# andrewmagis/snap-rnaseq

Measured on AMD Instinct MI355X. Metric: aligned reads/sec (100 bp SE, k=20 seed) at 1/2/4/8 GPUs + CPU baseline, higher is better.
Workload: dtype u8

## Files before the change

### snap-rnaseq_amd/csrc/aligner.hip

```cpp
#include <hip/hip_runtime.h>

#include <chrono>
#include <functional>
#include <cmath>
#include <cstring>
#include <algorithm>
#include <atomic>
#include <mutex>
#include <string>
#include <thread>
#include <type_traits>
#include <vector>

#include <fcntl.h>
#include <sys/stat.h>
#include <unistd.h>

#include "align_device.h"
#include "align_score.h"
#include "seed_lookup.h"
#include "simple_align.h"
#include "cigar.h"
#include "internal.h"
#include "large_copy.h"
// ... 973 lines not shown
uint32_t packedCode(char c) {
    return c == 'A' ? 0u : c == 'C' ? 1u : c == 'G' ? 2u : c == 'T' ? 3u : 4u;
}

int hostMapq(double pAll, double pBest, int score, int popular) {
    if (pAll < pBest) pAll = pBest;
    if (pAll == pBest && popular == 0 && score < 5) return 70;
    double c = pBest / pAll;
    int base;
    if (c >= 1) base = 69;
    else { base = (int)(-10 * log10(1 - c)); if (base > 69) base = 69; }
    int pen = popular - 10;
    if (pen < 0) pen = 0;
    base -= pen / 2;
    return base < 0 ? 0 : base;
}

}

struct ChunkSlot {
    char *dBases = nullptr, *dQuals = nullptr;
    uint64_t *dOffsets = nullptr;
    uint32_t *dLengths = nullptr;
    uint64_t *hOffsets = nullptr;
    uint32_t *hLengths = nullptr;
    snapgpu_result_t *hOut = nullptr;
    hipEvent_t h2d = nullptr;
    hipEvent_t done = nullptr;
    bool pending = false;
    uint64_t seq = 0, chunkBegin = 0, chunkN = 0, chunkEv = 0;
    snapgpu_result_t *chunkOut = nullptr;
};

struct ExecLane {
    hipStream_t stream = nullptr;
    void *arena = nullptr;
    void *bigArena = nullptr;
    uint32_t *counter = nullptr;
    unsigned long long *lookupStats = nullptr;
    hipEvent_t done = nullptr;
    uint64_t capReads = 0, capBytes = 0;
    uint32_t *dDefer = nullptr;
    snapgpu_result_t *dOut = nullptr;
    SeedRec *dSeeds = nullptr;
    ChunkSlot slot[2];
    uint32_t nextSlot = 0;
    unsigned long long *hLookupStats = nullptr;
};

struct EvSet {
    hipEvent_t e[4] = {};
    uint32_t *hCounter = nullptr;
};

struct SamState {
    struct Buf { void *p = nullptr; uint64_t cap = 0; };
    Buf aux;
    Buf len, scans, start, sums, text, bad;
    Buf bases, quals;
    Buf res, ed, nOps, ops;
    Buf key, keySorted, iota, order, slotLen, sortTemp;
    bool sorted = false;
    samline::SortArgs sortArgs{};
    std::vector<char> hAux;
    uint64_t fullBytes = 0;
    bool idsCached = false;
    std::string cachedRg;
    bool cachedHasRg = false;
    uint64_t n = 0, textBound = 0;
    bool ran = false;
    hipEvent_t ev[5] = {};
    double downloadMs = 0;
};

// ... 32 lines not shown

struct snapgpu_aligner {
    int device = 0;
    const snapgpu_index_t *idx = nullptr;
    snapgpu_aligner_params_t p{};
    uint32_t *dOverflow = nullptr, *dPieces = nullptr;
    uint4 *dBuckets = nullptr;
    uint64_t *dBucketBase = nullptr;
    uint32_t *dBucketCount = nullptr;
    snapgpu_bucket_info_t bucketInfo{};
    char *dGenomeAlloc = nullptr;
    GPlane *dGPlanes = nullptr;
    const char *dGenome = nullptr;
    DevTables *dTab = nullptr;
    ExecLane lane[2];
    std::vector<EvSet> evs;
    uint64_t nEvUsed = 0;
    bool overlapKernels = true;
    bool streamOpen = false;
    uint64_t nextLane = 0;
    uint64_t chunkSeq = 0;
    hipStream_t copyStream = nullptr;
    hipStream_t sideStream = nullptr;
    std::chrono::steady_clock::time_point streamStart;
    uint64_t arenaElems = 0;
    uint64_t arenaCap = 0;
    int grid = 0, grid256 = 0, grid512 = 0, gridBig = 0;
    uint64_t chunkReads = 1u << 20;
    uint64_t residentChunk = 1u << 18;
    uint32_t radixMin = SKCAP + 1;
    bool simplePass = true;
    int gridSimple = 0;
    bool orderLong = true;
    uint32_t tripRead = 0xffffffffu;
    snapgpu_timing_t timing{};
    snapgpu_aligner_stats_t stats{};
    snapgpu_device_reads_t *lastReads = nullptr;
    bool pendingTiming = false;
    uint32_t *dDiag = nullptr;
    unsigned long long *dPhase = nullptr;
    double timeoutSec = 0;
    bool failed = false;
    hipError_t (*eventQuery)(hipEvent_t) = hipEventQuery;
    hipEvent_t cev[2] = {};
    hipEvent_t residentSideDone = nullptr;
    bool residentSidePending = false;
// ... 325 lines not shown
        for (;;) {
            const hipError_t q = a->eventQuery(ev);
            if (q == hipSuccess) break;
            if (q != hipErrorNotReady) HIPCHK(q);
            if (std::chrono::duration<double>(std::chrono::steady_clock::now() - t0).count() > a->timeoutSec) {
                a->failed = true;
                snapgpu::setError("align kernel did not finish within SNAPGPU_TIMEOUT_S; the aligner is unusable "
                                  "and its device buffers are not released (exit the process)");
                return SNAPGPU_EDEVICE;
            }
            std::this_thread::sleep_for(std::chrono::microseconds(200));
        }
    }
    HIPCHK(hipEventSynchronize(ev));
    return SNAPGPU_OK;
}

int waitLane(snapgpu_aligner_t *a, ExecLane &L) {
    if (a->failed) return waitEvent(a, nullptr);
    HIPCHK(hipEventRecord(L.done, L.stream));
    return waitEvent(a, L.done);
}

}

namespace snapgpu {
void *hostAlloc(size_t bytes, bool *pinned, bool zero) {
    *pinned = false;
    int nd = g_hostDevices.load();
    if (nd == -2) {
        if (hipGetDeviceCount(&nd) != hipSuccess) nd = 0;
        g_hostDevices = nd;
    }
    if (nd > 0 && bytes >= (1u << 20)) {
        void *p = nullptr;
        size_t cap = bytes;
        {
            std::lock_guard<std::mutex> lk(g_pinMu);
            int best = -1;
            for (size_t i = 0; i < g_pinParked.size(); i++)
                if (g_pinParked[i].second >= bytes && g_pinParked[i].second <= 2 * bytes &&
                    (best < 0 || g_pinParked[i].second < g_pinParked[(size_t)best].second))
                    best = (int)i;
            if (best >= 0) {
                p = g_pinParked[(size_t)best].first;
                cap = g_pinParked[(size_t)best].second;
// ... 114 lines not shown
                                   idx->genome->nBases, a->dBuckets, a->dBucketBase, 4 * total);
                unsigned long long info[4] = {0, 0, 0, 0};
                if (chk(hipGetLastError(), "bucket_place_kernel / bucket_fill_kernel") &&
                    chk(hipMemcpyAsync(info, dCnt, sizeof(info), hipMemcpyDeviceToHost, s0), "counts") &&
                    chk(hipStreamSynchronize(s0), "bucket image build")) {
                    if (info[2] || info[0] != keys) {
                        snapgpu::setError("bucket image: " + std::to_string(info[2]) + " keys found no bucket, " +
                                          std::to_string(info[0]) + " of " + std::to_string(keys) + " inserted");
                        rc = SNAPGPU_EDEVICE;
                    }
                    snapgpu_bucket_info_t &bi = a->bucketInfo;
                    bi.nBuckets = total; bi.nKeys = info[0]; bi.nSlots = nSlots;
                    bi.nOverflowBuckets = info[1]; bi.maxDisplacement = info[3]; bi.bytes = total * 64;
                }
            }
        }
    }
    devFree(a, dSlots); devFree(a, dTB); devFree(a, dTS); devFree(a, dCnt);
    a->bucketInfo.buildMs = std::chrono::duration<double, std::milli>(std::chrono::steady_clock::now() - t0).count();
    return rc;
}

static void freeLaneChunkBuffers(snapgpu_aligner_t *a, ExecLane &L) {
    devFree(a, L.dDefer); devFree(a, L.dOut); devFree(a, L.dSeeds);
    L.dDefer = nullptr; L.dOut = nullptr; L.dSeeds = nullptr;
    for (ChunkSlot &S : L.slot) {
        devFree(a, S.dBases); devFree(a, S.dQuals); devFree(a, S.dOffsets); devFree(a, S.dLengths);
        S.dBases = S.dQuals = nullptr; S.dOffsets = nullptr; S.dLengths = nullptr;
        if (!a->failed) { hostPinnedFree(S.hOffsets); hostPinnedFree(S.hLengths); hostPinnedFree(S.hOut); }
        S.hOffsets = nullptr; S.hLengths = nullptr; S.hOut = nullptr;
    }
    L.capReads = L.capBytes = 0;
}

void snapgpu_aligner_free(snapgpu_aligner_t *a) {
    if (!a) return;
    if (a->failed) {
        delete a;
        return;
    }
    hipSetDevice(a->device);
    for (auto &L : a->lane) if (L.stream) hipStreamSynchronize(L.stream);
    devFree(a, a->dBuckets); devFree(a, a->dOverflow); devFree(a, a->dPieces);
    devFree(a, a->dBucketBase); devFree(a, a->dBucketCount); devFree(a, a->dGenomeAlloc); devFree(a, a->dTab);
    devFree(a, a->dGPlanes); devFree(a, a->dPhase); devFree(a, a->dDiag);
    for (auto &L : a->lane) {
        freeLaneChunkBuffers(a, L);
        devFree(a, L.arena); devFree(a, L.bigArena); devFree(a, L.counter); devFree(a, L.lookupStats);
        hostPinnedFree(L.hLookupStats);
        if (L.done) hipEventDestroy(L.done);
        for (ChunkSlot &S : L.slot) {
            if (S.h2d) hipEventDestroy(S.h2d);
            if (S.done) hipEventDestroy(S.done);
        }
        if (L.stream) hipStreamDestroy(L.stream);
    }
    if (a->copyStream) { hipStreamSynchronize(a->copyStream); hipStreamDestroy(a->copyStream); }
    if (a->sideStream) { hipStreamSynchronize(a->sideStream); hipStreamDestroy(a->sideStream); }
    for (auto &v : a->evs) {
        for (auto &e : v.e) if (e) hipEventDestroy(e);
        hostPinnedFree(v.hCounter);
    }
    for (auto &e : a->cev) if (e) hipEventDestroy(e);
    if (a->residentSideDone) hipEventDestroy(a->residentSideDone);
    for (auto *b : {&a->cgIn, &a->cgOut}) devFree(a, b->p);
    for (auto &b : a->aux) devFree(a, b.p);
    hostPinnedFree(a->cgPin);
    hostPinnedFree(a->cgPinOut);
    samStateFree(a, a->samBatch);
    bamStateFree(a, a->bamBatch);
    bgzfStateFree(a, a->bgzfBatch);
    for (int k = 0; k < 2; k++) {
        if (!a->failed) hostPinnedFree(a->samPin[k]);
        if (a->samPinDone[k]) hipEventDestroy(a->samPinDone[k]);
    }
    for (auto *b : {&a->fq.text, &a->fq.counts, &a->fq.tileStart, &a->fq.sums, &a->fq.nl, &a->fq.rec, &a->fq.baseStart,
                    &a->fq.idStart, &a->fq.sums2, &a->fq.tot, &a->fq.ids})
        devFree(a, b->p);
    for (int k = 0; k < 2; k++) {
        if (!a->failed) hostPinnedFree(a->fq.pin[k]);
        if (a->fq.pinDone[k]) hipEventDestroy(a->fq.pinDone[k]);
    }
    for (auto &e : a->fq.ev) if (e) hipEventDestroy(e);
// ... 16 lines not shown
    a->device = device;
    a->idx = idx;
    a->p = *params;
    if (const char *t = getenv("SNAPGPU_TIMEOUT_S")) a->timeoutSec = atof(t);
    if (const char *t = getenv("SNAPGPU_CHUNK_READS"); t && atoll(t) > 0) a->chunkReads = (uint64_t)atoll(t);
    if (const char *t = getenv("SNAPGPU_RADIX_MIN"); t && atoll(t) > 0) a->radixMin = (uint32_t)atoll(t);
    if (const char *t = getenv("SNAPGPU_OVERLAP")) a->overlapKernels = atoi(t) != 0;
    if (const char *t = getenv("SNAPGPU_ORDER_LONG")) a->orderLong = atoi(t) != 0;
    if (const char *t = getenv("SNAPGPU_SIMPLE_PASS")) a->simplePass = atoi(t) != 0;
    auto fail = [&](const char *what, hipError_t e) {
        snapgpu::setError(std::string(what) + ": " + hipGetErrorString(e));
        snapgpu_aligner_free(a);
        return (snapgpu_aligner_t *)nullptr;
    };
    hipError_t e;
    if ((e = hipSetDevice(device)) != hipSuccess) return fail("hipSetDevice", e);
    for (auto &L : a->lane) {
        if ((e = hipStreamCreateWithFlags(&L.stream, hipStreamNonBlocking)) != hipSuccess) return fail("stream", e);
        if ((e = hipEventCreateWithFlags(&L.done, hipEventDisableTiming)) != hipSuccess) return fail("event", e);
        for (ChunkSlot &S : L.slot)
            if ((e = hipEventCreateWithFlags(&S.h2d, hipEventDisableTiming)) != hipSuccess ||
                (e = hipEventCreateWithFlags(&S.done, hipEventDisableTiming)) != hipSuccess)
                return fail("event", e);
        if ((e = hipMalloc(&L.counter, 64)) != hipSuccess) return fail("counter", e);
        if ((e = hipMalloc(&L.lookupStats, 1024 * sizeof(unsigned long long))) != hipSuccess) return fail("lookup stats", e);
        if ((e = hipHostMalloc(&L.hLookupStats, 1024 * sizeof(unsigned long long), hipHostMallocDefault)) != hipSuccess)
            return fail("pinned lookup stats", e);
    }
    if ((e = hipStreamCreateWithFlags(&a->copyStream, hipStreamNonBlocking)) != hipSuccess) return fail("stream", e);
    {
        int least = 0, greatest = 0;
        const char *t = getenv("SNAPGPU_SIDE_PRIORITY");
        const bool high = !(t && atoi(t) == 0) && hipDeviceGetStreamPriorityRange(&least, &greatest) == hipSuccess;
        if ((e = high ? hipStreamCreateWithPriority(&a->sideStream, hipStreamNonBlocking, greatest)
                      : hipStreamCreateWithFlags(&a->sideStream, hipStreamNonBlocking)) != hipSuccess) return fail("stream", e);
    }
    for (auto &ev : a->cev) if ((e = hipEventCreate(&ev)) != hipSuccess) return fail("event", e);
    if ((e = hipEventCreateWithFlags(&a->residentSideDone, hipEventDisableTiming)) != hipSuccess) return fail("event", e);
    hipStream_t s0 = a->stream();
    if ((e = hipMalloc(&a->dDiag, 4 * sizeof(uint32_t))) != hipSuccess) return fail("watchdog record", e);
    if ((e = hipMemsetAsync(a->dDiag, 0, 4 * sizeof(uint32_t), s0)) != hipSuccess) return fail("watchdog record", e);
    if ((e = ensureDeviceTables(device)) != hipSuccess) return fail("device tables", e);
    const uint32_t nBases = idx->genome->nBases;
    const size_t gbytes = kDevGuard + nBases + kDevGuard;
    if ((e = hipMalloc(&a->dGenomeAlloc, gbytes)) != hipSuccess) return fail("hipMalloc genome", e);
    if ((e = hipMemsetAsync(a->dGenomeAlloc, 'n', gbytes, s0)) != hipSuccess) return fail("genome guard", e);
    if (uploadLarge(s0, a->dGenomeAlloc + kDevGuard, idx->genome->bases(), nBases)) { snapgpu_aligner_free(a); return nullptr; }
    a->dGenome = a->dGenomeAlloc + kDevGuard;
    {
        const uint64_t span = (uint64_t)nBases + 2 * kDevGuard;
        const uint64_t nw = (span + 31) / 32 + 8;
        if ((e = hipMalloc(&a->dGPlanes, nw * sizeof(GPlane))) != hipSuccess) return fail("hipMalloc planes", e);
        hipLaunchKernelGGL(pack_planes_kernel, dim3((unsigned)((nw + 255) / 256)), dim3(256), 0, s0, a->dGenomeAlloc,
                           span, nw, a->dGPlanes);
        if ((e = hipGetLastError()) != hipSuccess) return fail("pack_planes_kernel", e);
    }
    if ((e = hipMalloc(&a->dOverflow, idx->overflow.size() * 4 + 16)) != hipSuccess) return fail("hipMalloc ovf", e);
    if (uploadLarge(s0, a->dOverflow, idx->overflow.data(), idx->overflow.size() * 4)) { snapgpu_aligner_free(a); return nullptr; }
// ... 133 lines not shown

struct AlignExt {
    const snapgpu_search_t *search = nullptr;
    uint32_t maxHitsToGet = 0;
    uint32_t *hitScratch = nullptr;
    int32_t *multiFound = nullptr;
    snapgpu_multi_hit_t *multiHits = nullptr;
};

struct PassIO {
    const char *bases, *quals;
    const uint64_t *offsets;
    const uint32_t *lengths;
    uint64_t n;
    snapgpu_result_t *out;
    uint32_t *defer;
    uint32_t *defer2;
    uint32_t *ovf;
    SeedRec *seeds;
    uint32_t maxLen;
};

static int launch_passes(snapgpu_aligner_t *a, int li, const PassIO &io, const AlignExt &x, EvSet &ev,
                         const EvSet *prev) {
    ExecLane &L = a->lane[li];
    if (io.n == 0) return SNAPGPU_OK;
    if (io.n > 0xffffffffull) { snapgpu::setError("batch too large"); return SNAPGPU_EINVAL; }
    KArgs A;
    memset(&A, 0, sizeof(A));
    const snapgpu_index_t *idx = a->idx;
    A.buckets = a->dBuckets; A.bucketBase = a->dBucketBase; A.bucketCount = a->dBucketCount; A.overflow = a->dOverflow;
    A.genome = a->dGenome; A.pieces = a->dPieces; A.nPieces = (int32_t)idx->genome->pieceOffsets.size();
    A.gpl = a->dGPlanes; A.hasIupac = idx->hasIupac ? 1u : 0u;
    A.phaseBuf = a->dPhase;
    A.diag = a->dDiag;
    A.nBases = idx->genome->nBases; A.seedLen = idx->seedLen; A.nTables = idx->nTables;
    A.padding = idx->genome->chromosomePadding;
    A.maxHits = a->p.maxHitsToConsider; A.maxK = a->p.maxK; A.maxReadSize = a->p.maxReadSize;
    A.maxSeedsCmd = a->p.maxSeedsToUse; A.seedCoverage = a->p.maxSeedCoverage; A.extra = a->p.extraSearchDepth;
    A.explore = a->p.explorePopularSeeds; A.stopOnFirst = a->p.stopOnFirstHit; A.kRows = 31;
    A.radixMin = a->radixMin;
    A.tripRead = a->tripRead;
    A.tab = a->dTab;
    A.bases = io.bases; A.quals = io.quals; A.offsets = io.offsets; A.lengths = io.lengths;
    A.nReads = (uint32_t)io.n; A.out = io.out;
    A.counter = L.counter; A.arena = L.arena; A.arenaElems = a->arenaCap;
    if (a->arenaCap < a->arenaElems) { A.ovfList = io.ovf; A.ovfCount = L.counter + 6; }
    A.deferList = io.defer; A.deferCount = L.counter + 2; A.readList = nullptr;
    A.forcedStats = L.counter + 10;
    A.search = x.search; A.maxHitsToGet = x.maxHitsToGet;
    A.hitSlot = x.maxHitsToGet < 512 ? x.maxHitsToGet : 512;
    A.hitStride = multiHitStride(x.maxHitsToGet);
    A.hitScratch = x.hitScratch; A.multiFound = x.multiFound; A.multiHits = x.multiHits;
    int grid = a->grid;
    if ((uint64_t)grid > io.n) grid = (int)io.n;
    (void)hipGetLastError();
    if (prev && !a->overlapKernels) HIPCHK(hipStreamWaitEvent(L.stream, prev->e[2], 0));
    HIPCHK(hipMemsetAsync(L.counter, 0, 64, L.stream));
    HIPCHK(hipMemsetAsync(io.out, 0xff, io.n * sizeof(snapgpu_result_t), L.stream));
    A.seedRecs = nullptr;
    A.longCount = L.counter + 5;
    A.orderTmp = a->orderLong && io.n < (1ull << 28) ? io.defer2 : nullptr;
    HIPCHK(hipEventRecord(ev.e[3], L.stream));
    hipLaunchKernelGGL(seed_lookup_kernel, dim3((unsigned)((io.n + 4 * LOOKUP_WAVES - 1) / (4 * LOOKUP_WAVES))),
                       dim3(64 * LOOKUP_WAVES), 0, L.stream, A, io.seeds,
                       L.lookupStats);
    HIPCHK(hipGetLastError());
    if (A.orderTmp && io.maxLen > 128) {
        hipLaunchKernelGGL(order_long_kernel, dim3(1), dim3(256), 0, L.stream, A.orderTmp, A.longCount, A.deferList);
        HIPCHK(hipGetLastError());
    }
    A.orderTmp = nullptr;
    A.seedRecs = reinterpret_cast<const uint4 *>(io.seeds);
    HIPCHK(hipEventRecord(ev.e[0], L.stream));
    const bool ext = x.search || x.maxHitsToGet;
    if (a->simplePass && !ext && !A.stopOnFirst && !A.explore && A.maxHits >= 1 && A.maxHits < 0xffffu && A.seedRecs &&
        !A.phaseBuf) {
        KArgs Q = A;
        Q.counter = L.counter + 8;
        int gridS = a->gridSimple;
        if ((uint64_t)gridS > io.n) gridS = (int)io.n;
        if ((uint64_t)gridS * SIMPLE_CHUNK > io.n) gridS = (int)((io.n + SIMPLE_CHUNK - 1) / SIMPLE_CHUNK);
        hipLaunchKernelGGL(simple_align_kernel, dim3(gridS), dim3(64), 0, L.stream, Q, io.defer2, L.counter + 9,
                           L.counter + 12, L.counter + 13);
        HIPCHK(hipGetLastError());
        A.readList = io.defer2; A.readCount = L.counter + 9;
    }
    if (ext) hipLaunchKernelGGL((align_kernel<128, true>), dim3(grid), dim3(64), 0, L.stream, A);
    else hipLaunchKernelGGL((align_kernel<128, false>), dim3(grid), dim3(64), 0, L.stream, A);
    HIPCHK(hipGetLastError());
    HIPCHK(hipEventRecord(ev.e[1], L.stream));
    A.readList = nullptr; A.readCount = nullptr;
    KArgs M = A;
    M.counter = L.counter + 3;
    M.readList = io.defer; M.readCount = L.counter + 2;
    M.deferList = io.defer2; M.deferCount = L.counter + 4;
    int grid256 = a->grid256;
    if ((uint64_t)grid256 > io.n) grid256 = (int)io.n;
    if (ext) hipLaunchKernelGGL((align_kernel<256, true>), dim3(grid256), dim3(64), 0, L.stream, M);
    else hipLaunchKernelGGL((align_kernel<256, false>), dim3(grid256), dim3(64), 0, L.stream, M);
    HIPCHK(hipGetLastError());
    KArgs B = A;
    B.counter = L.counter + 1;
    B.readList = io.defer2; B.readCount = L.counter + 4;
    B.deferList = nullptr; B.deferCount = nullptr;
    B.seedRecs = nullptr;
    int grid2 = a->grid512;
    if ((uint64_t)grid2 > io.n) grid2 = (int)io.n;
    if (ext) hipLaunchKernelGGL((align_kernel<512, true>), dim3(grid2), dim3(64), 0, L.stream, B);
    else hipLaunchKernelGGL((align_kernel<512, false>), dim3(grid2), dim3(64), 0, L.stream, B);
    HIPCHK(hipGetLastError());
    if (a->gridBig) {
        KArgs V = A;
        V.counter = L.counter + 7;
        V.readList = io.ovf; V.readCount = L.counter + 6;
        V.deferList = nullptr; V.deferCount = nullptr;
        V.ovfList = nullptr; V.ovfCount = nullptr;
        V.seedRecs = nullptr;
        V.arena = L.bigArena; V.arenaElems = a->arenaElems;
        int gridV = a->gridBig;
        if ((uint64_t)gridV > io.n) gridV = (int)io.n;
        if (ext) hipLaunchKernelGGL((align_kernel<512, true>), dim3(gridV), dim3(64), 0, L.stream, V);
        else hipLaunchKernelGGL((align_kernel<512, false>), dim3(gridV), dim3(64), 0, L.stream, V);
        HIPCHK(hipGetLastError());
    }
    HIPCHK(hipEventRecord(ev.e[2], L.stream));
    HIPCHK(hipMemcpyAsync(ev.hCounter, L.counter, 64, hipMemcpyDeviceToHost, L.stream));
    return SNAPGPU_OK;
}

static EvSet *nextEvSet(snapgpu_aligner_t *a) {
    if (a->nEvUsed == a->evs.size()) {
        EvSet v;
        for (auto &e : v.e)
            if (hipEventCreate(&e) != hipSuccess) { snapgpu::setError("hipEventCreate"); return nullptr; }
        if (hipHostMalloc(&v.hCounter, 64, hipHostMallocDefault) != hipSuccess) { snapgpu::setError("pinned counter"); return nullptr; }
        a->evs.push_back(v);
    }
    return &a->evs[a->nEvUsed++];
}

static int beginCall(snapgpu_aligner_t *a) {
    a->nEvUsed = 0;
    a->timing = snapgpu_timing_t{};
    for (auto &L : a->lane) HIPCHK(hipMemsetAsync(L.lookupStats, 0, 1024 * sizeof(unsigned long long), L.stream));
    HIPCHK(hipMemsetAsync(a->dDiag, 0, sizeof(uint32_t) * 4, a->lane[0].stream));
    HIPCHK(hipStreamSynchronize(a->lane[0].stream));
    return SNAPGPU_OK;
}

static double busyUnion(snapgpu_aligner_t *a, int from, int to) {
    std::vector<std::pair<float, float>> iv;
    const hipEvent_t ref = a->evs[0].e[3];
    for (uint64_t i = 0; i < a->nEvUsed; i++) {
        float b = 0, e = 0;
        if (hipEventElapsedTime(&b, ref, a->evs[i].e[from]) != hipSuccess ||
            hipEventElapsedTime(&e, ref, a->evs[i].e[to]) != hipSuccess) return -1;
        iv.emplace_back(b, e);
    }
    std::sort(iv.begin(), iv.end());
    double total = 0, cs = -1e30, ce = -1e30;
    for (auto &x : iv) {
        if (x.first > ce) { if (ce > cs) total += ce - cs; cs = x.first; ce = x.second; }
        else if (x.second > ce) ce = x.second;
    }
    if (ce > cs) total += ce - cs;
    return total;
}

static void accountBusy(snapgpu_aligner_t *a) {
    if (a->nEvUsed == 0) return;
    a->timing.mainKernelBusyMs = busyUnion(a, 0, 1);
    a->timing.lookupKernelBusyMs = busyUnion(a, 3, 0);
}

static int accountEvSet(snapgpu_aligner_t *a, const EvSet &v) {
    float ms = 0;
    HIPCHK(hipEventElapsedTime(&ms, v.e[0], v.e[1]));
    a->timing.mainKernelMs += ms;
    HIPCHK(hipEventElapsedTime(&ms, v.e[1], v.e[2]));
    a->timing.spillKernelMs += ms;
    HIPCHK(hipEventElapsedTime(&ms, v.e[3], v.e[0]));
    a->timing.lookupKernelMs += ms;
    a->timing.nLaunches++;
    a->timing.nSpilled += v.hCounter[2];
    a->timing.nByteReads += v.hCounter[4];
    a->timing.nArenaOverflow += v.hCounter[6];
    a->timing.nForcedSettled += v.hCounter[10];
    a->timing.nForcedLimitSpans += v.hCounter[11];
    a->timing.nSimpleBailed += v.hCounter[9];
    a->timing.nSimpleReads += v.hCounter[12];
    a->timing.nSimpleWide += v.hCounter[13];
    return SNAPGPU_OK;
}

int snapgpu_align_batch_wait(snapgpu_aligner_t *a);

static int launch_resident(snapgpu_aligner_t *a, snapgpu_device_reads_t *d, const AlignExt &x) {
    if (!a || !d) return SNAPGPU_EINVAL;
    if (a->failed) { snapgpu::setError("aligner failed earlier (device timeout)"); return SNAPGPU_EDEVICE; }
    HIPCHK(hipSetDevice(a->device));
    int rc = snapgpu_align_batch_wait(a);
    if (rc) return rc;
    rc = beginCall(a);
    if (rc) return rc;
    if (a->residentSidePending) {
        for (auto &L : a->lane) HIPCHK(hipStreamWaitEvent(L.stream, a->residentSideDone, 0));
        a->residentSidePending = false;
    }
    const bool ext = x.search || x.maxHitsToGet;
    const uint64_t n = d->n;
    const uint64_t nChunks = ext || n == 0 ? 1 : (n + a->residentChunk - 1) / a->residentChunk;
    const uint64_t per = (n + nChunks - 1) / nChunks;
    for (uint64_t c = 0; c < nChunks; c++) {
        const uint64_t b = c * per, m = std::min(n, b + per) - b;
        EvSet *ev = nextEvSet(a);
        if (!ev) return SNAPGPU_EDEVICE;
        PassIO io{d->dBases, d->dQuals, d->dOffsets + b, d->dLengths + b, m, d->dOut + b, d->dDefer + b,
                  d->dDefer + (n + 1) + b, d->dDefer + 2 * (n + 1) + b, d->dSeeds + b * SEEDS_PER_READ, d->maxLen};
        if ((rc = launch_passes(a, (int)(c & 1), io, x, *ev, c ? &a->evs[a->nEvUsed - 2] : nullptr))) return rc;
    }
    a->lastReads = d;
    a->pendingTiming = n > 0;
    return SNAPGPU_OK;
}

int snapgpu_align_resident(snapgpu_aligner_t *a, snapgpu_device_reads_t *d) { return launch_resident(a, d, AlignExt()); }

static void addLookupStats(snapgpu_timing_t &t, const unsigned long long *ls) {
    for (int i = 0; i < 256; i++) {
        t.lookupSeeds += ls[4 * i];
        t.lookupProbes += ls[4 * i + 1];
        t.lookupOverflowReads += ls[4 * i + 2];
    }
}

static int checkWatchdog(snapgpu_aligner_t *a) {
    uint32_t diag[4];
    HIPCHK(hipMemcpy(diag, a->dDiag, sizeof(diag), hipMemcpyDeviceToHost));
    if (diag[0]) {
        char msg[160];
        snprintf(msg, sizeof msg, "device watchdog tripped: code %u read %u detail %u", diag[0], diag[1], diag[2]);
        snapgpu::setError(msg);
        return SNAPGPU_EDEVICE;
    }
    return SNAPGPU_OK;
}

int snapgpu_synchronize(snapgpu_aligner_t *a) {
    if (!a) return SNAPGPU_EINVAL;
    if (a->failed) { snapgpu::setError("aligner failed earlier (device timeout)"); return SNAPGPU_EDEVICE; }
    HIPCHK(hipSetDevice(a->device));
    for (auto &L : a->lane) {
        const int rc = waitLane(a, L);
        if (rc) return rc;
    }
    if (a->pendingTiming) {
        a->timing = snapgpu_timing_t{};
        for (uint64_t i = 0; i < a->nEvUsed; i++) {
            const int rc = accountEvSet(a, a->evs[i]);
            if (rc) return rc;
        }
        accountBusy(a);
        std::vector<unsigned long long> ls(1024);
        for (auto &L : a->lane) {
            HIPCHK(hipMemcpy(ls.data(), L.lookupStats, 1024 * sizeof(unsigned long long), hipMemcpyDeviceToHost));
            addLookupStats(a->timing, ls.data());
        }
        a->pendingTiming = false;
        const int rc = checkWatchdog(a);
        if (rc) return rc;
    }
    return SNAPGPU_OK;
}

static int checkRecords(snapgpu_aligner_t *a, uint64_t unwritten, uint64_t firstUnwritten) {
    a->timing.nUnwritten += unwritten;
    if (!unwritten) return SNAPGPU_OK;
    if (int rc = checkWatchdog(a)) return rc;
// ... 24 lines not shown
    return checkRecords(a, unwritten, first);
}

int snapgpu_results_download(snapgpu_aligner_t *a, snapgpu_device_reads_t *d, snapgpu_result_t *out) {
    if (!a || !d || !out) return SNAPGPU_EINVAL;
    HIPCHK(hipSetDevice(a->device));
    int rc = snapgpu_synchronize(a);
    if (rc) return rc;
    HIPCHK(hipMemcpyAsync(out, d->dOut, d->n * sizeof(snapgpu_result_t), hipMemcpyDeviceToHost, a->stream()));
    HIPCHK(hipStreamSynchronize(a->stream()));
    auto t0 = std::chrono::steady_clock::now();
    a->timing.nMapqFixed = 0;
    a->timing.nNulReads = 0;
    a->timing.nUnwritten = 0;
    rc = finishRecords(a, out, d->n);
    a->timing.fixupMs = std::chrono::duration<double, std::milli>(std::chrono::steady_clock::now() - t0).count();
    return rc;
}

static int ensureLaneCapacity(snapgpu_aligner_t *a, ExecLane &L, uint64_t reads, uint64_t bytes) {
    if (reads <= L.capReads && bytes <= L.capBytes) return SNAPGPU_OK;
    int rc = waitLane(a, L);
    if (rc) return rc;
    freeLaneChunkBuffers(a, L);
    reads = std::max<uint64_t>(reads, 1024);
    const uint64_t cb = bytes + 512;
    for (ChunkSlot &S : L.slot) {
        HIPCHK(hipMalloc(&S.dBases, cb));
        HIPCHK(hipMalloc(&S.dQuals, cb));
        HIPCHK(hipMemsetAsync(S.dBases, 0, cb, a->copyStream));
        HIPCHK(hipMemsetAsync(S.dQuals, 0, cb, a->copyStream));
        HIPCHK(hipMalloc(&S.dOffsets, (reads + 1) * 8));
        HIPCHK(hipMalloc(&S.dLengths, (reads + 1) * 4));
        HIPCHK(hipHostMalloc(&S.hOffsets, (reads + 1) * 8, hipHostMallocDefault));
        HIPCHK(hipHostMalloc(&S.hLengths, (reads + 1) * 4, hipHostMallocDefault));
        HIPCHK(hipHostMalloc(&S.hOut, (reads + 1) * sizeof(snapgpu_result_t), hipHostMallocDefault));
    }
    HIPCHK(hipMalloc(&L.dDefer, 3 * (reads + 1) * 4));
    HIPCHK(hipMalloc(&L.dOut, (reads + 1) * sizeof(snapgpu_result_t)));
    HIPCHK(hipMalloc(&L.dSeeds, (reads + 8) * SEEDS_PER_READ * sizeof(SeedRec)));
    L.capReads = reads;
    L.capBytes = bytes;
    return SNAPGPU_OK;
}

static int finishChunk(snapgpu_aligner_t *a, ChunkSlot &L) {
    if (!L.pending) return SNAPGPU_OK;
    snapgpu_result_t *out = L.chunkOut;
    L.pending = false;
    int rc = waitEvent(a, L.done);
    if (rc) return rc;
    if ((rc = accountEvSet(a, a->evs[L.chunkEv]))) return rc;
    const auto t0 = std::chrono::steady_clock::now();
    const uint64_t n = L.chunkN;
    snapgpu_result_t *dst = out + L.chunkBegin;
    const unsigned nt = n >= 65536 ? snapgpu::hostThreads(4) : 1u;
    std::vector<snapgpu_aligner_stats_t> st(nt, snapgpu_aligner_stats_t{});
    std::vector<uint64_t> fixed(nt, 0), nul(nt, 0), unwritten(nt, 0), first(nt, 0);
    auto work = [&](unsigned t) {
        const uint64_t b = n * t / nt, e = n * (t + 1) / nt;
        memcpy(dst + b, L.hOut + b, (e - b) * sizeof(snapgpu_result_t));
        uint64_t lk = 0, sc = 0, ig = 0, tm = 0, fx = 0, nu = 0, uw = 0, f0 = 0;
        for (uint64_t i = b; i < e; i++) {
// ... 42 lines not shown

static int finishOldest(snapgpu_aligner_t *a, bool *any) {
    ChunkSlot *o = nullptr;
    for (auto &L : a->lane)
        for (ChunkSlot &S : L.slot)
            if (S.pending && (!o || S.seq < o->seq)) o = &S;
    *any = o != nullptr;
    return o ? finishChunk(a, *o) : SNAPGPU_OK;
}

static int finishAll(snapgpu_aligner_t *a) {
    for (bool any = true; any;) {
        const int rc = finishOldest(a, &any);
        if (rc) return rc;
    }
    return SNAPGPU_OK;
}

static void abandonChunks(snapgpu_aligner_t *a) {
    for (auto &L : a->lane) {
        for (ChunkSlot &S : L.slot) S.pending = false;
        if (!a->failed) waitLane(a, L);
    }
    if (!a->failed && a->copyStream) (void)hipStreamSynchronize(a->copyStream);
    a->streamOpen = false;
}

int snapgpu_align_batch_submit(snapgpu_aligner_t *a, const snapgpu_reads_t *reads, snapgpu_result_t *out) {
    if (!a || !reads || !out) return SNAPGPU_EINVAL;
    if (a->failed) { snapgpu::setError("aligner failed earlier (device timeout)"); return SNAPGPU_EDEVICE; }
    HIPCHK(hipSetDevice(a->device));
    int rc = SNAPGPU_OK;
    if (!a->streamOpen) {
        if (a->pendingTiming && (rc = snapgpu_synchronize(a))) return rc;
        if ((rc = beginCall(a))) return rc;
        a->streamOpen = true;
        a->streamStart = std::chrono::steady_clock::now();
    }
    const uint64_t n = reads->n;
    if (n == 0) return SNAPGPU_OK;
    const uint64_t nChunks = (n + a->chunkReads - 1) / a->chunkReads;
    const uint64_t per = (n + nChunks - 1) / nChunks;
    std::vector<uint64_t> lo(nChunks, ~0ull), hi(nChunks, 0);
    uint64_t maxSpan = 0;
    for (uint64_t c = 0; c < nChunks; c++) {
        for (uint64_t i = c * per; i < std::min(n, (c + 1) * per); i++) {
// ... 14 lines not shown
    for (uint64_t c = 0; c < nChunks && rc == SNAPGPU_OK; c++) {
        const int li = (int)(a->nextLane++ & 1);
        ExecLane &L = a->lane[li];
        ChunkSlot &S = L.slot[L.nextSlot];
        L.nextSlot ^= 1u;
        for (bool any = true; S.pending && any;)
            if ((rc = finishOldest(a, &any))) break;
        if (rc) break;
        const uint64_t b = c * per, m = std::min(n, b + per) - b;
        uint32_t maxLen = 0;
        for (uint64_t i = 0; i < m; i++) {
            S.hOffsets[i] = reads->offsets[b + i] - lo[c];
            const uint32_t ln = reads->lengths[b + i];
            S.hLengths[i] = ln;
            maxLen = std::max(maxLen, ln);
        }
        const uint64_t span = std::min(hi[c] + 64, std::max(hostEnd, hi[c])) - lo[c];
        hipStream_t cs = a->copyStream, s = L.stream;
        HIPBRK(hipMemcpyAsync(S.dBases, reads->bases + lo[c], span, hipMemcpyHostToDevice, cs));
        HIPBRK(hipMemcpyAsync(S.dQuals, reads->quals + lo[c], span, hipMemcpyHostToDevice, cs));
        HIPBRK(hipMemcpyAsync(S.dOffsets, S.hOffsets, m * 8, hipMemcpyHostToDevice, cs));
        HIPBRK(hipMemcpyAsync(S.dLengths, S.hLengths, m * 4, hipMemcpyHostToDevice, cs));
        HIPBRK(hipEventRecord(S.h2d, cs));
        HIPBRK(hipStreamWaitEvent(s, S.h2d, 0));
        PassIO io{S.dBases, S.dQuals, S.dOffsets, S.dLengths, m, L.dOut, L.dDefer, L.dDefer + (L.capReads + 1),
                  L.dDefer + 2 * (L.capReads + 1), L.dSeeds, maxLen};
        EvSet *ev = nextEvSet(a);
        if (!ev) { rc = SNAPGPU_EDEVICE; break; }
        if ((rc = launch_passes(a, li, io, AlignExt(), *ev, a->nEvUsed >= 2 ? &a->evs[a->nEvUsed - 2] : nullptr))) break;
        HIPBRK(hipMemcpyAsync(S.hOut, L.dOut, m * sizeof(snapgpu_result_t), hipMemcpyDeviceToHost, s));
        HIPBRK(hipEventRecord(S.done, s));
        S.pending = true;
        S.seq = a->chunkSeq++;
        S.chunkBegin = b;
        S.chunkN = m;
        S.chunkEv = a->nEvUsed - 1;
        S.chunkOut = out;
    }
    if (rc) abandonChunks(a);
    return rc;
}

int snapgpu_align_batch_wait(snapgpu_aligner_t *a) {
    if (!a) return SNAPGPU_EINVAL;
    if (!a->streamOpen) return a->failed ? SNAPGPU_EDEVICE : SNAPGPU_OK;
    HIPCHK(hipSetDevice(a->device));
    int rc = finishAll(a);
    a->streamOpen = false;
    if (rc) {
        abandonChunks(a);
        return rc;
    }
    accountBusy(a);
// ... 1733 lines not shown
            rc = SNAPGPU_EDEVICE;
        }
    }
    devFree(a, dS); devFree(a, dO); devFree(a, dL);
    return rc;
}

int snapgpu_aligner_bucket_info(const snapgpu_aligner_t *a, snapgpu_bucket_info_t *info) {
    if (!a || !info) return SNAPGPU_EINVAL;
    *info = a->bucketInfo;
    return SNAPGPU_OK;
}

int snapgpu_gather_peak(snapgpu_aligner_t *a, uint32_t nLoads, double *ms) {
    if (!a || !ms || nLoads == 0) return SNAPGPU_EINVAL;
    HIPCHK(hipSetDevice(a->device));
    const uint64_t nBk = a->bucketInfo.nBuckets;
    if (nBk == 0 || nBk >= (1ull << 32)) { snapgpu::setError("gather_peak: bucket count"); return SNAPGPU_EINVAL; }
    const unsigned grid = (nLoads + 1023) / 1024;
    float best = 0;
    for (int rep = 0; rep < 3; rep++) {
        HIPCHK(hipEventRecord(a->cev[0], a->stream()));
        hipLaunchKernelGGL(gather_peak_kernel, dim3(grid), dim3(256), 0, a->stream(), a->dBuckets, (uint32_t)nBk, nLoads,
                           0x5bd1e995u * (rep + 1), a->lane[0].counter + 8);
        HIPCHK(hipGetLastError());
        HIPCHK(hipEventRecord(a->cev[1], a->stream()));
        HIPCHK(hipEventSynchronize(a->cev[1]));
        float f = 0;
        HIPCHK(hipEventElapsedTime(&f, a->cev[0], a->cev[1]));
        if (rep == 0 || f < best) best = f;
    }
    *ms = best;
    return SNAPGPU_OK;
}

int snapgpu_copy_peak(snapgpu_aligner_t *a, uint64_t bytes, double *ms) {
    if (!a || !ms || bytes < 4096) return SNAPGPU_EINVAL;
    if (a->failed) return SNAPGPU_EDEVICE;
    HIPCHK(hipSetDevice(a->device));
    const uint64_t nw = bytes / 16 / 1024 * 1024;
    void *src = nullptr, *dst = nullptr;
    HIPCHK(hipMalloc(&src, nw * 16));
    if (hipMalloc(&dst, nw * 16) != hipSuccess) { devFree(a, src); snapgpu::setError("copy_peak: hipMalloc"); return SNAPGPU_ENOMEM; }
    hipDeviceProp_t prop;
    HIPCHK(hipGetDeviceProperties(&prop, a->device));
    const unsigned grid = (unsigned)prop.multiProcessorCount * 16;
    float best = 0;
// ... 54 lines not shown
```

Measured before the change: 62.57 million.

## Run seed lookup and simple pass on a shared front stream with per-slot buffers

Seed lookup, order_long and simple_align now run on a new shared front stream that waits on the chunk's H2D event. The main align passes stay on the lane streams and wait on the front stream through an event, so lookup for the next chunk can overlap alignment of the previous one. To make that safe, the output, defer and seed buffers move from each lane to each chunk slot, and the device counters move to each event set. Separately, the 256 and 512 align passes are skipped when the reads are at most 128 bp and the index has no IUPAC codes, removing two kernel launches for short reads. The cost is more device memory, extra event and stream synchronisation, and the front stream serialising lookup work across both lanes.

Result: faster. 65.06 million (median of 6 runs) (+4.0%).

```diff
diff --git a/snap-rnaseq_amd/csrc/aligner.hip b/snap-rnaseq_amd/csrc/aligner.hip
--- a/snap-rnaseq_amd/csrc/aligner.hip
+++ b/snap-rnaseq_amd/csrc/aligner.hip
@@ -1019,6 +1019,9 @@
     char *dBases = nullptr, *dQuals = nullptr;
     uint64_t *dOffsets = nullptr;
     uint32_t *dLengths = nullptr;
+    uint32_t *dDefer = nullptr;
+    snapgpu_result_t *dOut = nullptr;
+    SeedRec *dSeeds = nullptr;
     uint64_t *hOffsets = nullptr;
     uint32_t *hLengths = nullptr;
     snapgpu_result_t *hOut = nullptr;
@@ -1033,20 +1036,17 @@
     hipStream_t stream = nullptr;
     void *arena = nullptr;
     void *bigArena = nullptr;
-    uint32_t *counter = nullptr;
     unsigned long long *lookupStats = nullptr;
     hipEvent_t done = nullptr;
     uint64_t capReads = 0, capBytes = 0;
-    uint32_t *dDefer = nullptr;
-    snapgpu_result_t *dOut = nullptr;
-    SeedRec *dSeeds = nullptr;
     ChunkSlot slot[2];
     uint32_t nextSlot = 0;
     unsigned long long *hLookupStats = nullptr;
 };
 
 struct EvSet {
-    hipEvent_t e[4] = {};
+    hipEvent_t e[6] = {};
+    uint32_t *dCounter = nullptr;
     uint32_t *hCounter = nullptr;
 };
 
@@ -1125,6 +1125,9 @@
     uint64_t chunkSeq = 0;
     hipStream_t copyStream = nullptr;
     hipStream_t sideStream = nullptr;
+    hipStream_t frontStream = nullptr;
+    hipEvent_t frontDone = nullptr;
+    uint32_t *dSink = nullptr;
     std::chrono::steady_clock::time_point streamStart;
     uint64_t arenaElems = 0;
     uint64_t arenaCap = 0;
@@ -1496,6 +1499,12 @@
     return waitEvent(a, L.done);
 }
 
+int waitFront(snapgpu_aligner_t *a) {
+    if (a->failed) return waitEvent(a, nullptr);
+    HIPCHK(hipEventRecord(a->frontDone, a->frontStream));
+    return waitEvent(a, a->frontDone);
+}
+
 }
 
 namespace snapgpu {
@@ -1656,9 +1665,9 @@
 }
 
 static void freeLaneChunkBuffers(snapgpu_aligner_t *a, ExecLane &L) {
-    devFree(a, L.dDefer); devFree(a, L.dOut); devFree(a, L.dSeeds);
-    L.dDefer = nullptr; L.dOut = nullptr; L.dSeeds = nullptr;
     for (ChunkSlot &S : L.slot) {
+        devFree(a, S.dDefer); devFree(a, S.dOut); devFree(a, S.dSeeds);
+        S.dDefer = nullptr; S.dOut = nullptr; S.dSeeds = nullptr;
         devFree(a, S.dBases); devFree(a, S.dQuals); devFree(a, S.dOffsets); devFree(a, S.dLengths);
         S.dBases = S.dQuals = nullptr; S.dOffsets = nullptr; S.dLengths = nullptr;
         if (!a->failed) { hostPinnedFree(S.hOffsets); hostPinnedFree(S.hLengths); hostPinnedFree(S.hOut); }
@@ -1674,13 +1683,14 @@
         return;
     }
     hipSetDevice(a->device);
+    if (a->frontStream) hipStreamSynchronize(a->frontStream);
     for (auto &L : a->lane) if (L.stream) hipStreamSynchronize(L.stream);
     devFree(a, a->dBuckets); devFree(a, a->dOverflow); devFree(a, a->dPieces);
     devFree(a, a->dBucketBase); devFree(a, a->dBucketCount); devFree(a, a->dGenomeAlloc); devFree(a, a->dTab);
     devFree(a, a->dGPlanes); devFree(a, a->dPhase); devFree(a, a->dDiag);
     for (auto &L : a->lane) {
         freeLaneChunkBuffers(a, L);
-        devFree(a, L.arena); devFree(a, L.bigArena); devFree(a, L.counter); devFree(a, L.lookupStats);
+        devFree(a, L.arena); devFree(a, L.bigArena); devFree(a, L.lookupStats);
         hostPinnedFree(L.hLookupStats);
         if (L.done) hipEventDestroy(L.done);
         for (ChunkSlot &S : L.slot) {
@@ -1691,8 +1701,12 @@
     }
     if (a->copyStream) { hipStreamSynchronize(a->copyStream); hipStreamDestroy(a->copyStream); }
     if (a->sideStream) { hipStreamSynchronize(a->sideStream); hipStreamDestroy(a->sideStream); }
+    if (a->frontStream) hipStreamDestroy(a->frontStream);
+    if (a->frontDone) hipEventDestroy(a->frontDone);
+    devFree(a, a->dSink);
     for (auto &v : a->evs) {
         for (auto &e : v.e) if (e) hipEventDestroy(e);
+        devFree(a, v.dCounter);
         hostPinnedFree(v.hCounter);
     }
     for (auto &e : a->cev) if (e) hipEventDestroy(e);
@@ -1755,7 +1769,6 @@
             if ((e = hipEventCreateWithFlags(&S.h2d, hipEventDisableTiming)) != hipSuccess ||
                 (e = hipEventCreateWithFlags(&S.done, hipEventDisableTiming)) != hipSuccess)
                 return fail("event", e);
-        if ((e = hipMalloc(&L.counter, 64)) != hipSuccess) return fail("counter", e);
         if ((e = hipMalloc(&L.lookupStats, 1024 * sizeof(unsigned long long))) != hipSuccess) return fail("lookup stats", e);
         if ((e = hipHostMalloc(&L.hLookupStats, 1024 * sizeof(unsigned long long), hipHostMallocDefault)) != hipSuccess)
             return fail("pinned lookup stats", e);
@@ -1767,6 +1780,12 @@
         const bool high = !(t && atoi(t) == 0) && hipDeviceGetStreamPriorityRange(&least, &greatest) == hipSuccess;
         if ((e = high ? hipStreamCreateWithPriority(&a->sideStream, hipStreamNonBlocking, greatest)
                       : hipStreamCreateWithFlags(&a->sideStream, hipStreamNonBlocking)) != hipSuccess) return fail("stream", e);
+        const char *f = getenv("SNAPGPU_FRONT_PRIORITY");
+        const bool fhigh = f && atoi(f) != 0 && hipDeviceGetStreamPriorityRange(&least, &greatest) == hipSuccess;
+        if ((e = fhigh ? hipStreamCreateWithPriority(&a->frontStream, hipStreamNonBlocking, greatest)
+                       : hipStreamCreateWithFlags(&a->frontStream, hipStreamNonBlocking)) != hipSuccess) return fail("stream", e);
+        if ((e = hipEventCreateWithFlags(&a->frontDone, hipEventDisableTiming)) != hipSuccess) return fail("event", e);
+        if ((e = hipMalloc(&a->dSink, 64)) != hipSuccess) return fail("sink", e);
     }
     for (auto &ev : a->cev) if ((e = hipEventCreate(&ev)) != hipSuccess) return fail("event", e);
     if ((e = hipEventCreateWithFlags(&a->residentSideDone, hipEventDisableTiming)) != hipSuccess) return fail("event", e);
@@ -1946,8 +1965,10 @@
 };
 
 static int launch_passes(snapgpu_aligner_t *a, int li, const PassIO &io, const AlignExt &x, EvSet &ev,
-                         const EvSet *prev) {
+                         const EvSet *prev, hipEvent_t inputs = nullptr, bool front = true) {
     ExecLane &L = a->lane[li];
+    uint32_t *const cnt = ev.dCounter;
+    const hipStream_t fs = front ? a->frontStream : L.stream;
     if (io.n == 0) return SNAPGPU_OK;
     if (io.n > 0xffffffffull) { snapgpu::setError("batch too large"); return SNAPGPU_EINVAL; }
     KArgs A;
@@ -1968,10 +1989,10 @@
     A.tab = a->dTab;
     A.bases = io.bases; A.quals = io.quals; A.offsets = io.offsets; A.lengths = io.lengths;
     A.nReads = (uint32_t)io.n; A.out = io.out;
-    A.counter = L.counter; A.arena = L.arena; A.arenaElems = a->arenaCap;
-    if (a->arenaCap < a->arenaElems) { A.ovfList = io.ovf; A.ovfCount = L.counter + 6; }
-    A.deferList = io.defer; A.deferCount = L.counter + 2; A.readList = nullptr;
-    A.forcedStats = L.counter + 10;
+    A.counter = cnt; A.arena = L.arena; A.arenaElems = a->arenaCap;
+    if (a->arenaCap < a->arenaElems) { A.ovfList = io.ovf; A.ovfCount = cnt + 6; }
+    A.deferList = io.defer; A.deferCount = cnt + 2; A.readList = nullptr;
+    A.forcedStats = cnt + 10;
     A.search = x.search; A.maxHitsToGet = x.maxHitsToGet;
     A.hitSlot = x.maxHitsToGet < 512 ? x.maxHitsToGet : 512;
     A.hitStride = multiHitStride(x.maxHitsToGet);
@@ -1979,65 +2000,73 @@
     int grid = a->grid;
     if ((uint64_t)grid > io.n) grid = (int)io.n;
     (void)hipGetLastError();
-    if (prev && !a->overlapKernels) HIPCHK(hipStreamWaitEvent(L.stream, prev->e[2], 0));
-    HIPCHK(hipMemsetAsync(L.counter, 0, 64, L.stream));
-    HIPCHK(hipMemsetAsync(io.out, 0xff, io.n * sizeof(snapgpu_result_t), L.stream));
+    if (prev && !a->overlapKernels) HIPCHK(hipStreamWaitEvent(fs, prev->e[2], 0));
+    if (inputs) HIPCHK(hipStreamWaitEvent(fs, inputs, 0));
+    HIPCHK(hipMemsetAsync(cnt, 0, 64, fs));
+    HIPCHK(hipMemsetAsync(io.out, 0xff, io.n * sizeof(snapgpu_result_t), fs));
     A.seedRecs = nullptr;
-    A.longCount = L.counter + 5;
+    A.longCount = cnt + 5;
     A.orderTmp = a->orderLong && io.n < (1ull << 28) ? io.defer2 : nullptr;
-    HIPCHK(hipEventRecord(ev.e[3], L.stream));
+    HIPCHK(hipEventRecord(ev.e[3], fs));
     hipLaunchKernelGGL(seed_lookup_kernel, dim3((unsigned)((io.n + 4 * LOOKUP_WAVES - 1) / (4 * LOOKUP_WAVES))),
-                       dim3(64 * LOOKUP_WAVES), 0, L.stream, A, io.seeds,
+                       dim3(64 * LOOKUP_WAVES), 0, fs, A, io.seeds,
                        L.lookupStats);
     HIPCHK(hipGetLastError());
     if (A.orderTmp && io.maxLen > 128) {
-        hipLaunchKernelGGL(order_long_kernel, dim3(1), dim3(256), 0, L.stream, A.orderTmp, A.longCount, A.deferList);
+        hipLaunchKernelGGL(order_long_kernel, dim3(1), dim3(256), 0, fs, A.orderTmp, A.longCount, A.deferList);
         HIPCHK(hipGetLastError());
     }
     A.orderTmp = nullptr;
     A.seedRecs = reinterpret_cast<const uint4 *>(io.seeds);
-    HIPCHK(hipEventRecord(ev.e[0], L.stream));
+    HIPCHK(hipEventRecord(ev.e[0], fs));
     const bool ext = x.search || x.maxHitsToGet;
     if (a->simplePass && !ext && !A.stopOnFirst && !A.explore && A.maxHits >= 1 && A.maxHits < 0xffffu && A.seedRecs &&
         !A.phaseBuf) {
         KArgs Q = A;
-        Q.counter = L.counter + 8;
+        Q.counter = cnt + 8;
         int gridS = a->gridSimple;
         if ((uint64_t)gridS > io.n) gridS = (int)io.n;
         if ((uint64_t)gridS * SIMPLE_CHUNK > io.n) gridS = (int)((io.n + SIMPLE_CHUNK - 1) / SIMPLE_CHUNK);
-        hipLaunchKernelGGL(simple_align_kernel, dim3(gridS), dim3(64), 0, L.stream, Q, io.defer2, L.counter + 9,
-                           L.counter + 12, L.counter + 13);
+        hipLaunchKernelGGL(simple_align_kernel, dim3(gridS), dim3(64), 0, fs, Q, io.defer2, cnt + 9,
+                           cnt + 12, cnt + 13);
         HIPCHK(hipGetLastError());
-        A.readList = io.defer2; A.readCount = L.counter + 9;
-    }
+        A.readList = io.defer2; A.readCount = cnt + 9;
+    }
+    HIPCHK(hipEventRecord(ev.e[4], fs));
+    HIPCHK(hipStreamWaitEvent(L.stream, ev.e[4], 0));
+    HIPCHK(hipEventRecord(ev.e[5], L.stream));
     if (ext) hipLaunchKernelGGL((align_kernel<128, true>), dim3(grid), dim3(64), 0, L.stream, A);
     else hipLaunchKernelGGL((align_kernel<128, false>), dim3(grid), dim3(64), 0, L.stream, A);
     HIPCHK(hipGetLastError());
     HIPCHK(hipEventRecord(ev.e[1], L.stream));
     A.readList = nullptr; A.readCount = nullptr;
+    const bool pass2 = io.maxLen > 128 || idx->hasIupac;
+    const bool pass3 = pass2 && (io.maxLen > 256 || idx->hasIupac);
     KArgs M = A;
-    M.counter = L.counter + 3;
-    M.readList = io.defer; M.readCount = L.counter + 2;
-    M.deferList = io.defer2; M.deferCount = L.counter + 4;
+    M.counter = cnt + 3;
+    M.readList = io.defer; M.readCount = cnt + 2;
+    M.deferList = io.defer2; M.deferCount = cnt + 4;
     int grid256 = a->grid256;
     if ((uint64_t)grid256 > io.n) grid256 = (int)io.n;
-    if (ext) hipLaunchKernelGGL((align_kernel<256, true>), dim3(grid256), dim3(64), 0, L.stream, M);
+    if (!pass2) {}
+    else if (ext) hipLaunchKernelGGL((align_kernel<256, true>), dim3(grid256), dim3(64), 0, L.stream, M);
     else hipLaunchKernelGGL((align_kernel<256, false>), dim3(grid256), dim3(64), 0, L.stream, M);
     HIPCHK(hipGetLastError());
     KArgs B = A;
-    B.counter = L.counter + 1;
-    B.readList = io.defer2; B.readCount = L.counter + 4;
+    B.counter = cnt + 1;
+    B.readList = io.defer2; B.readCount = cnt + 4;
     B.deferList = nullptr; B.deferCount = nullptr;
     B.seedRecs = nullptr;
     int grid2 = a->grid512;
     if ((uint64_t)grid2 > io.n) grid2 = (int)io.n;
-    if (ext) hipLaunchKernelGGL((align_kernel<512, true>), dim3(grid2), dim3(64), 0, L.stream, B);
+    if (!pass3) {}
+    else if (ext) hipLaunchKernelGGL((align_kernel<512, true>), dim3(grid2), dim3(64), 0, L.stream, B);
     else hipLaunchKernelGGL((align_kernel<512, false>), dim3(grid2), dim3(64), 0, L.stream, B);
     HIPCHK(hipGetLastError());
     if (a->gridBig) {
         KArgs V = A;
-        V.counter = L.counter + 7;
-        V.readList = io.ovf; V.readCount = L.counter + 6;
+        V.counter = cnt + 7;
+        V.readList = io.ovf; V.readCount = cnt + 6;
         V.deferList = nullptr; V.deferCount = nullptr;
         V.ovfList = nullptr; V.ovfCount = nullptr;
         V.seedRecs = nullptr;
@@ -2049,7 +2078,7 @@
         HIPCHK(hipGetLastError());
     }
     HIPCHK(hipEventRecord(ev.e[2], L.stream));
-    HIPCHK(hipMemcpyAsync(ev.hCounter, L.counter, 64, hipMemcpyDeviceToHost, L.stream));
+    HIPCHK(hipMemcpyAsync(ev.hCounter, cnt, 64, hipMemcpyDeviceToHost, L.stream));
     return SNAPGPU_OK;
 }
 
@@ -2058,6 +2087,7 @@
         EvSet v;
         for (auto &e : v.e)
             if (hipEventCreate(&e) != hipSuccess) { snapgpu::setError("hipEventCreate"); return nullptr; }
+        if (hipMalloc(&v.dCounter, 64) != hipSuccess) { snapgpu::setError("device counter"); return nullptr; }
         if (hipHostMalloc(&v.hCounter, 64, hipHostMallocDefault) != hipSuccess) { snapgpu::setError("pinned counter"); return nullptr; }
         a->evs.push_back(v);
     }
@@ -2069,11 +2099,15 @@
     a->timing = snapgpu_timing_t{};
     for (auto &L : a->lane) HIPCHK(hipMemsetAsync(L.lookupStats, 0, 1024 * sizeof(unsigned long long), L.stream));
     HIPCHK(hipMemsetAsync(a->dDiag, 0, sizeof(uint32_t) * 4, a->lane[0].stream));
+    for (auto &L : a->lane) {
+        HIPCHK(hipEventRecord(L.done, L.stream));
+        HIPCHK(hipStreamWaitEvent(a->frontStream, L.done, 0));
+    }
     HIPCHK(hipStreamSynchronize(a->lane[0].stream));
     return SNAPGPU_OK;
 }
 
-static double busyUnion(snapgpu_aligner_t *a, int from, int to) {
+static double busyUnion(snapgpu_aligner_t *a, int from, int to, int from2 = -1, int to2 = -1) {
     std::vector<std::pair<float, float>> iv;
     const hipEvent_t ref = a->evs[0].e[3];
     for (uint64_t i = 0; i < a->nEvUsed; i++) {
@@ -2081,6 +2115,10 @@
         if (hipEventElapsedTime(&b, ref, a->evs[i].e[from]) != hipSuccess ||
             hipEventElapsedTime(&e, ref, a->evs[i].e[to]) != hipSuccess) return -1;
         iv.emplace_back(b, e);
+        if (from2 < 0) continue;
+        if (hipEventElapsedTime(&b, ref, a->evs[i].e[from2]) != hipSuccess ||
+            hipEventElapsedTime(&e, ref, a->evs[i].e[to2]) != hipSuccess) return -1;
+        iv.emplace_back(b, e);
     }
     std::sort(iv.begin(), iv.end());
     double total = 0, cs = -1e30, ce = -1e30;
@@ -2094,13 +2132,15 @@
 
 static void accountBusy(snapgpu_aligner_t *a) {
     if (a->nEvUsed == 0) return;
-    a->timing.mainKernelBusyMs = busyUnion(a, 0, 1);
+    a->timing.mainKernelBusyMs = busyUnion(a, 0, 4, 5, 1);
     a->timing.lookupKernelBusyMs = busyUnion(a, 3, 0);
 }
 
 static int accountEvSet(snapgpu_aligner_t *a, const EvSet &v) {
     float ms = 0;
-    HIPCHK(hipEventElapsedTime(&ms, v.e[0], v.e[1]));
+    HIPCHK(hipEventElapsedTime(&ms, v.e[0], v.e[4]));
+    a->timing.mainKernelMs += ms;
+    HIPCHK(hipEventElapsedTime(&ms, v.e[5], v.e[1]));
     a->timing.mainKernelMs += ms;
     HIPCHK(hipEventElapsedTime(&ms, v.e[1], v.e[2]));
     a->timing.spillKernelMs += ms;
@@ -2129,6 +2169,7 @@
     rc = beginCall(a);
     if (rc) return rc;
     if (a->residentSidePending) {
+        HIPCHK(hipStreamWaitEvent(a->frontStream, a->residentSideDone, 0));
         for (auto &L : a->lane) HIPCHK(hipStreamWaitEvent(L.stream, a->residentSideDone, 0));
         a->residentSidePending = false;
     }
@@ -2142,7 +2183,8 @@
         if (!ev) return SNAPGPU_EDEVICE;
         PassIO io{d->dBases, d->dQuals, d->dOffsets + b, d->dLengths + b, m, d->dOut + b, d->dDefer + b,
                   d->dDefer + (n + 1) + b, d->dDefer + 2 * (n + 1) + b, d->dSeeds + b * SEEDS_PER_READ, d->maxLen};
-        if ((rc = launch_passes(a, (int)(c & 1), io, x, *ev, c ? &a->evs[a->nEvUsed - 2] : nullptr))) return rc;
+        if ((rc = launch_passes(a, (int)(c & 1), io, x, *ev, c ? &a->evs[a->nEvUsed - 2] : nullptr, nullptr, false)))
+            return rc;
     }
     a->lastReads = d;
     a->pendingTiming = n > 0;
@@ -2179,6 +2221,7 @@
         const int rc = waitLane(a, L);
         if (rc) return rc;
     }
+    if (const int rc = waitFront(a)) return rc;
     if (a->pendingTiming) {
         a->timing = snapgpu_timing_t{};
         for (uint64_t i = 0; i < a->nEvUsed; i++) {
@@ -2249,6 +2292,7 @@
     if (reads <= L.capReads && bytes <= L.capBytes) return SNAPGPU_OK;
     int rc = waitLane(a, L);
     if (rc) return rc;
+    if ((rc = waitFront(a))) return rc;
     freeLaneChunkBuffers(a, L);
     reads = std::max<uint64_t>(reads, 1024);
     const uint64_t cb = bytes + 512;
@@ -2262,10 +2306,10 @@
         HIPCHK(hipHostMalloc(&S.hOffsets, (reads + 1) * 8, hipHostMallocDefault));
         HIPCHK(hipHostMalloc(&S.hLengths, (reads + 1) * 4, hipHostMallocDefault));
         HIPCHK(hipHostMalloc(&S.hOut, (reads + 1) * sizeof(snapgpu_result_t), hipHostMallocDefault));
-    }
-    HIPCHK(hipMalloc(&L.dDefer, 3 * (reads + 1) * 4));
-    HIPCHK(hipMalloc(&L.dOut, (reads + 1) * sizeof(snapgpu_result_t)));
-    HIPCHK(hipMalloc(&L.dSeeds, (reads + 8) * SEEDS_PER_READ * sizeof(SeedRec)));
+        HIPCHK(hipMalloc(&S.dDefer, 3 * (reads + 1) * 4));
+        HIPCHK(hipMalloc(&S.dOut, (reads + 1) * sizeof(snapgpu_result_t)));
+        HIPCHK(hipMalloc(&S.dSeeds, (reads + 8) * SEEDS_PER_READ * sizeof(SeedRec)));
+    }
     L.capReads = reads;
     L.capBytes = bytes;
     return SNAPGPU_OK;
@@ -2354,6 +2398,7 @@
         for (ChunkSlot &S : L.slot) S.pending = false;
         if (!a->failed) waitLane(a, L);
     }
+    if (!a->failed) waitFront(a);
     if (!a->failed && a->copyStream) (void)hipStreamSynchronize(a->copyStream);
     a->streamOpen = false;
 }
@@ -2414,13 +2459,12 @@
         HIPBRK(hipMemcpyAsync(S.dOffsets, S.hOffsets, m * 8, hipMemcpyHostToDevice, cs));
         HIPBRK(hipMemcpyAsync(S.dLengths, S.hLengths, m * 4, hipMemcpyHostToDevice, cs));
         HIPBRK(hipEventRecord(S.h2d, cs));
-        HIPBRK(hipStreamWaitEvent(s, S.h2d, 0));
-        PassIO io{S.dBases, S.dQuals, S.dOffsets, S.dLengths, m, L.dOut, L.dDefer, L.dDefer + (L.capReads + 1),
-                  L.dDefer + 2 * (L.capReads + 1), L.dSeeds, maxLen};
+        PassIO io{S.dBases, S.dQuals, S.dOffsets, S.dLengths, m, S.dOut, S.dDefer, S.dDefer + (L.capReads + 1),
+                  S.dDefer + 2 * (L.capReads + 1), S.dSeeds, maxLen};
         EvSet *ev = nextEvSet(a);
         if (!ev) { rc = SNAPGPU_EDEVICE; break; }
-        if ((rc = launch_passes(a, li, io, AlignExt(), *ev, a->nEvUsed >= 2 ? &a->evs[a->nEvUsed - 2] : nullptr))) break;
-        HIPBRK(hipMemcpyAsync(S.hOut, L.dOut, m * sizeof(snapgpu_result_t), hipMemcpyDeviceToHost, s));
+        if ((rc = launch_passes(a, li, io, AlignExt(), *ev, a->nEvUsed >= 2 ? &a->evs[a->nEvUsed - 2] : nullptr, S.h2d))) break;
+        HIPBRK(hipMemcpyAsync(S.hOut, S.dOut, m * sizeof(snapgpu_result_t), hipMemcpyDeviceToHost, s));
         HIPBRK(hipEventRecord(S.done, s));
         S.pending = true;
         S.seq = a->chunkSeq++;
@@ -4200,7 +4244,7 @@
     for (int rep = 0; rep < 3; rep++) {
         HIPCHK(hipEventRecord(a->cev[0], a->stream()));
         hipLaunchKernelGGL(gather_peak_kernel, dim3(grid), dim3(256), 0, a->stream(), a->dBuckets, (uint32_t)nBk, nLoads,
-                           0x5bd1e995u * (rep + 1), a->lane[0].counter + 8);
+                           0x5bd1e995u * (rep + 1), a->dSink + 8);
         HIPCHK(hipGetLastError());
         HIPCHK(hipEventRecord(a->cev[1], a->stream()));
         HIPCHK(hipEventSynchronize(a->cev[1]));
```
